# roboyu/Kimera-Multi

Measured on AMD Instinct MI355X. Metric: dpgo edges*iters/sec (+ LC candidates verified/sec in 'lcd'), higher is better.
Workload: dtype f64

## Files before the change

### kimera-multi_amd/csrc/pgo.hip

```cpp
#include <hip/hip_runtime.h>
#include <hip/hip_ext.h>
#include <rccl/rccl.h>
#include <dlfcn.h>

#include <algorithm>
#include <chrono>
#include <thread>
#include <type_traits>
#include <cmath>
#include <cstdio>
#include <cstdlib>
#include <cstring>
#include <limits>
#include <numeric>
#include <string>
#include <vector>

#include "common.h"
#include "pgo_host.h"

#ifndef KMX_HESS_PROBE
#define KMX_HESS_PROBE 0
#endif

// ... 201 lines not shown
  static constexpr int WK = RW == 10 ? 6 : 12;
  static constexpr int QS = RW == 10 ? 4 : Q;
  __device__ static __forceinline__ void load_stored(const Dev& d, size_t k, double2 a[QS]) {
    const double2* p2 = reinterpret_cast<const double2*>(d.rec + (size_t)GS * k);
#pragma unroll
    for (int i = 0; i < QS; ++i) a[i] = p2[i];
  }
  __device__ static __forceinline__ unsigned load_word(const Dev& d, size_t k) {
    static_assert(RW == 10, "compact records only");
    return (unsigned)d.rec_o[k];
  }
  __device__ static __forceinline__ int other_of(unsigned word) {
    static_assert(RW == 10, "compact records only");
    return (int)(word << 3) >> 3;
  }
  __device__ static __forceinline__ void expand(const double2 a[QS], unsigned raw, double2 q[Q]) {
    if constexpr (RW == 10) {
      const double2 a0 = a[0], a1 = a[1], a2 = a[2], a3 = a[3];
      const int other = (int)(raw << 3) >> 3;
      const unsigned big = raw >> 29;
      const double qa = a0.x, qb = a0.y, qc = a1.x;
      const double ql = sqrt(1.0 - (qa * qa + qb * qb + qc * qc));
      const double w = big == 0 ? ql : qa, x = big == 0 ? qa : (big == 1 ? ql : qb);
      const double y = big <= 1 ? qb : (big == 2 ? ql : qc), z = big == 3 ? ql : qc;
      q[0] = make_double2(w, x);
      q[1] = make_double2(y, z);
      q[2] = make_double2(a1.y, a2.x);
      q[3] = make_double2(a2.y, a3.x);
      const double wt = a3.y;
      const long long bits = (long long)(unsigned)other | (std::signbit(wt) ? (1ll << 63) : 0ll);
      q[4] = make_double2(std::fabs(wt), __longlong_as_double(bits));
    } else {
#pragma unroll
      for (int i = 0; i < Q; ++i) q[i] = a[i];
    }
// ... 473 lines not shown
__device__ __forceinline__ double inc_owner_cost(const Dev& d, const Lane& L, const double* V, const double* pub,
                                                 char* smem) {
  using SM = SmemC<R>;
  using RC = Rec<RW>;
  int* sptr = reinterpret_cast<int*>(smem + SM::ptr_off);
  double2* xs = reinterpret_cast<double2*>(smem + SM::x_off);
  const int tid = threadIdx.x;
  const int p0 = L.p0, np = L.np, K0 = L.k0, n = L.n;
  if (tid <= np) sptr[tid] = d.inc_ptr[p0 + tid] - K0;
  {
    const double2* v2 = reinterpret_cast<const double2*>(V + (size_t)p0 * 4 * R);
    for (int i = tid; i < np * 2 * R; i += BLOCK) xs[i] = v2[i];
  }
  __syncthreads();
  double cost = 0.0;
  for (int k = tid; k < n; k += BLOCK) {
    double2 q[RC::Q];
    RC::load(d, (size_t)(K0 + k), q);
    const int2 in = RC::inc(q);
    const int o = in.x;
    const bool tail = (in.y >> 31) & 1;
    if (o >= 0 && !tail) continue;
    const double2* o2 =
        reinterpret_cast<const double2*>((o >= 0) ? V + (size_t)o * 4 * R : pub + (size_t)(-1 - o) * 4 * R);
    double2 vs2[2 * R], vo2[2 * R];
#pragma unroll
    for (int i = 0; i < 2 * R; ++i) vo2[i] = o2[i];
    int lo = 0, hi = np;
    while (hi - lo > 1) {
      const int mid = (lo + hi) >> 1;
// ... 446 lines not shown

template <int R, int RW, int RM>
__device__ __forceinline__ void body_grad(const Dev& d, int gated, char* smem) {
  const Lane L = lane_map<R>(d);
  if (gated) {
    if (L.tile == 0 && threadIdx.x == 0) store_gnc(d.gnc, load_gnc(d.gnc_next));
    if (d.gnc_next->fired) {
      const int np = L.np, p0 = L.p0;
      for (int t = threadIdx.x; t < np; t += blockDim.x) pose_precond<RW>(d, p0 + t);
      __syncthreads();
    }
  }
  if (d.ctl[L.l].phase != PH_START) return;
  double y[4] = {0, 0, 0, 0}, G[4], cost = 0.0;
  hinc_grad<R, RW>(d, L, d.X, d.pub, G, &cost, smem);
  if (L.valid) load4(d.X + (size_t)L.pose * 4 * R + 4 * L.a, y);
  constexpr int NDP = R >= 5 ? 1 : 2;
  double2 dpart[NDP];
  {
    const double2* Dp2 = reinterpret_cast<const double2*>(d.hD + SYM4 * (size_t)L.pose);
#pragma unroll
    for (int u = 0; u < NDP; ++u) {
      const int i = L.a + u * R;
      dpart[u] = (L.valid && i < 5) ? Dp2[i] : make_double2(0.0, 0.0);
    }
  }
  double S[9], gr[4], zr[4];
  double* scr = reinterpret_cast<double*>(smem);
  group_symYtG<R, true>(y, G, L.base, S, scr);
#pragma unroll
  for (int c = 0; c < 3; ++c) gr[c] = G[c] - (y[0] * S[0 * 3 + c] + y[1] * S[1 * 3 + c] + y[2] * S[2 * 3 + c]);
  gr[3] = G[3];
  group_precon<R, true>(d, L.pose, L.valid, y, gr, L.base, zr, scr);
  double vals[3] = {cost, 0.0, 0.0};
  if (L.valid) {
    vals[1] = gr[0] * gr[0] + gr[1] * gr[1] + gr[2] * gr[2] + gr[3] * gr[3];
    vals[2] = zr[0] * gr[0] + zr[1] * gr[1] + zr[2] * gr[2] + zr[3] * gr[3];
  }
  finish_tile<RED_GRAD, 3, RM>(d, L, vals, smem + SmemHG<R>::red_off, [&]() {
    if (!L.valid) return;
    const size_t o = (size_t)L.pose * 4 * R + 4 * L.a;
    store4(d.g + o, gr);
    store4(d.z + o, zr);
    if (L.a == 0) {
      double* Sp = d.S + 6 * (size_t)L.pose;
      Sp[0] = S[0]; Sp[1] = S[1]; Sp[2] = S[2]; Sp[3] = S[4]; Sp[4] = S[5]; Sp[5] = S[8];
    }
    double2* Fp2 = reinterpret_cast<double2*>(d.hDS + SYM4 * (size_t)L.pose);
#pragma unroll
    for (int u = 0; u < NDP; ++u) {
      const int i = L.a + u * R;
      if (i < 5) {
        const double sx = i == 0 ? S[0] : i == 1 ? S[2] : i == 2 ? S[4] : 0.0;
        const double sy = i == 0 ? S[1] : i == 2 ? S[5] : i == 3 ? S[8] : 0.0;
        Fp2[i] = make_double2(dpart[u].x - sx, dpart[u].y - sy);
      }
    }
  });
}
// ... 700 lines not shown
      if (threadIdx.x == 0) {
        if (u.stop >= 0) d.ctl[L.l].tcg_stop = u.stop;
        d.ctl[L.l].phase = PH_STEP;
      }
    }
  }
}

template <int R>
__device__ __forceinline__ void body_commit(const Dev& d, int fold, int final) {
  const Lane L = lane_map<R>(d);
  if (final && L.tile == 0 && threadIdx.x == 0) {
    d.gnc->inner += 1;
    d.gnc->rounds += 1;
  }
  bool commit;
  if (fold) {
    __shared__ int sph;
    __shared__ Ctl cs;
    __shared__ double rl[NPART * WAVES];
    const Ctl& c = d.ctl[L.l];
    const bool writer = L.tile == L.rt0;
    if (writer && threadIdx.x < (int)(sizeof(Ctl) / 8))
      reinterpret_cast<double*>(&cs)[threadIdx.x] = reinterpret_cast<const double*>(&c)[threadIdx.x];
    if (threadIdx.x == 0) sph = c.phase;
    __syncthreads();
    if (sph != PH_STEP) return;
    RobotSum<NPART> rs;
    rs.issue(d.part, NPART, L.rt0, L.rt1);
    double tot[NPART] = {0.0, 0.0, 0.0, 0.0};
    rs.finish(d.part, NPART, rl, tot);
    if (d.p.rgd) {
      commit = true;
    } else {
      const double model_dec = -0.5 * tot[2];
      const double rho = (model_dec > 0.0) ? (c.f_cur - tot[0]) / model_dec : -1.0;
      commit = rho > d.p.accept_rho;
    }
    if (threadIdx.x == 0 && writer) {
      control_on(cs, d, L.l, RED_COST, tot, R, true);
      cs.phase = PH_STEP;
      d.ctl[L.l] = cs;
    }
  } else {
    const Ctl& c = d.ctl[L.l];
    commit = c.commit != 0;
    if (final && !commit && c.chg_acc > 0.0 && L.valid) {
      const int s = d.pose_slot[L.pose];
      if (s >= 0) {
        const size_t o = (size_t)L.pose * 4 * R + 4 * L.a;
        double v[4];
        load4(d.X + o, v);
        store4(d.pub + (size_t)s * 4 * R + 4 * L.a, v);
      }
    }
  }
  if (!commit || !L.valid) return;
  const size_t o = (size_t)L.pose * 4 * R + 4 * L.a;
  double v[4];
  load4(d.Xt + o, v);
  store4(d.X + o, v);
  if (!final) return;
  const int s = d.pose_slot[L.pose];
  if (s >= 0) store4(d.pub + (size_t)s * 4 * R + 4 * L.a, v);
}

template <int R, int RW, int RM>
__global__ __launch_bounds__(BLOCK, LB<R>::w) void k_grad(Dev d, int gated) {
  KMX_SMEM;
  body_grad<R, RW, RM>(d, gated, smem);
}
template <int R, int RW, int RM, bool GRAD, bool EARLY>
__global__ __launch_bounds__(BLOCK, LB<R>::w) void k_hess(Dev d, int gated, int slot, HostStatus* hs,
                                                          unsigned long long seq) {
// ... 515 lines not shown
  static constexpr int MAX_GROUPS = 4;
  struct Group {
    int l0 = 0, l1 = 0;
    int t0 = 0, nt = 0;
    int blind_left = 0;
  };
  int groups_req = 2;
  std::vector<Group> grp;
  Group all;
  int grm = 2;
  int grm_forced = -1;
  hipStream_t gstream[MAX_GROUPS - 1] = {nullptr, nullptr, nullptr};
  hipEvent_t ev_fork = nullptr, ev_join[MAX_GROUPS - 1] = {nullptr, nullptr, nullptr};
  bool hess_gate = true;
  bool tcg_tail = true;
  int rm = RM_LAUNCH;
  int rm_forced = -1;
  int early_stop = 1;
  int decide_forced = -1;
  bool poll_timeout = false;
  bool timing = false;
  int* d_hv_launch = nullptr;
  std::vector<hipEvent_t> ev_pool;
  size_t ev_used = 0;
  double *d_accV = nullptr, *d_accY = nullptr;
  double* d_X0 = nullptr;
  double acc_gamma = 0.0;
  int acc_k = 0;
  bool acc_ready = false, acc_started = false;
};
// ... 98 lines not shown
  p.mu_step = h->P.gnc_mu_step;
  p.rel_tol = h->gnc_rel_tol;
  p.gnc_on = h->gnc_on;
  p.inner_iters = h->gnc_inner_iters;
  p.max_updates = h->gnc_max_updates;
  p.n_ext = h->n_ext;
  p.rgd = h->P.method == KMX_METHOD_RGD ? 1 : 0;
  p.rgd_step = h->P.rgd_stepsize;
  h->dv.ext = h->d_ext;
}

void enqueue_publish(kmx_pgo* h) {
  const int ps = 4 * h->P.r;
  const long long tot = h->n_owned * ps;
  if (tot == 0) return;
  hipLaunchKernelGGL(k_publish, dim3((unsigned)((tot / 2 + 255) / 256)), dim3(256), 0, h->stream, h->d_vec,
                     h->d_pub + (size_t)h->first_owned * ps, h->d_pub_src + h->first_owned, (int)h->n_owned, ps);
}

void enqueue_precond(kmx_pgo* h, int gated) {
  const int blocks = std::max(1, std::min(gated ? 256 : 1024, (h->nloc + 127) / 128));
  with_rw(h->rw, [&](auto RW) {
    hipLaunchKernelGGL(k_precond<RW()>, dim3(blocks), dim3(128), 0, h->stream, h->dv, gated);
  });
}

bool enqueue_begin(kmx_pgo* h, const unsigned char* d_active, int mode, bool defer = false,
                   hipEvent_t done = nullptr) {
  const bool may_fire = h->P.robust_cost == KMX_COST_GNC_TLS && (h->gnc_on || (mode & BEGIN_FORCE_GNC));
  if (!may_fire) mode |= BEGIN_SOLO;
  const unsigned grid = may_fire ? 1 + (unsigned)std::min(256, std::max(1, (h->n_gnc + 255) / 256)) : 1;
// ... 189 lines not shown
    if (t.e0)
      hipExtLaunchKernelGGL((k_step<R, RW>), grid, blk, SmemF<R>::bytes, q.s, t.e0, t.e1, 0u, q.d, cin, cout, j,
                            t.slot, hs, seq);
    else
      hipLaunchKernelGGL((k_step<R, RW>), grid, blk, SmemF<R>::bytes, q.s, q.d, cin, cout, j, t.slot, hs, seq);
    if (poll && j > 0 && !wait_running(h, seq, q.l0, q.l0 + q.nl)) {
      J = j + 1;
      break;
    }
  }
  h->ctl_par = J & 1;
  tcg_polled(h, *q.st, poll, J - 1);
}

template <int R, int RW, int RM>
void enqueue_round_t(kmx_pgo* h, const unsigned char* d_active, int G) {
  constexpr bool cons = RM == RM_CONSUMER;
  const dim3 blk(BLOCK);
  const bool rgd = h->P.method == KMX_METHOD_RGD, os = cons && onesync(h);
  if (multi_rtr(h))
    (void)hipMemcpyAsync(h->d_X0, h->dv.X, sizeof(double) * (size_t)h->dv.vec, hipMemcpyDeviceToDevice, h->stream);
  const bool pend = enqueue_begin(h, d_active, BEGIN_ROUND, true, G > 1 ? h->ev_fork : nullptr);
  Chain q[kmx_pgo::MAX_GROUPS];
  if (G == 1) q[0] = make_chain(h, h->all, h->stream);
  else
    for (int g = 0; g < G; ++g) q[g] = make_chain(h, h->grp[g], g == 0 ? h->stream : h->gstream[g - 1]);
  for (int g = 1; g < G; ++g) (void)hipStreamWaitEvent(q[g].s, h->ev_fork, 0);
  const int iters = rgd ? 1 : h->P.rtr_iterations;
  const bool fgrad = fold_grad<RM>(h), fcost = fold_cost<RM>(h);
  for (int it = 0; it < iters; ++it) {
    for (int g = 0; g < G; ++g) {
// ... 12 lines not shown
      const bool last = it + 1 == iters;
      hipEvent_t join = g > 0 && last ? h->ev_join[g - 1] : nullptr;
      if (!os && !(cons && stopped[g]) && !tail_fused<RM>(h))
        hipLaunchKernelGGL((k_retract<R>), grid, blk, SmemU::bytes, q[g].s, q[g].d, cons && !rgd ? 2 : 0,
                           (const Ctl*)h->d_ctl);
      if (fcost && join)
        hipExtLaunchKernelGGL((k_cost<R, RW, RM>), grid, blk, SmemC<R>::bytes, q[g].s, nullptr, join, 0u, q[g].d, src);
      else
        hipLaunchKernelGGL((k_cost<R, RW, RM>), grid, blk, SmemC<R>::bytes, q[g].s, q[g].d, src);
      if (!fcost) red<R>(q[g], RED_COST, nullptr, 0, -1, join);
      if (!last)
        hipLaunchKernelGGL((k_commit<R>), grid, blk, 0, q[g].s, q[g].d, 0, 0);
    }
  }
  for (int g = 1; g < G; ++g) (void)hipStreamWaitEvent(h->stream, h->ev_join[g - 1], 0);
  hipLaunchKernelGGL((k_commit<R>), dim3(h->ntiles), blk, 0, h->stream, h->dv, fcost ? 1 : 0, 1);
  if (multi_rtr(h))
    hipLaunchKernelGGL(k_change, dim3(h->dv.L), blk, 0, h->stream, h->dv, (const double*)h->d_X0, 4 * R);
}

void enqueue_round(kmx_pgo* h, const unsigned char* d_active) {
  const int G = groups_in_effect(h);
  const int rm = G > 1 ? h->grm : h->rm;
  with_r(h->P.r, [&](auto R) {
    constexpr int r = decltype(R)::value;
    if (rm == RM_CONSUMER)
      with_rw(h->rw, [&](auto RW) { enqueue_round_t<r, RW(), RM_CONSUMER>(h, d_active, G); });
    else
      with_rw(h->rw, [&](auto RW) { enqueue_round_t<r, RW(), RM_LAUNCH>(h, d_active, G); });
  });
}

double accel_gamma_next(const kmx_pgo* h) {
  const double N = (double)h->n_robots;
  return (1.0 + std::sqrt(1.0 + 4.0 * N * N * h->acc_gamma * h->acc_gamma)) / (2.0 * N);
}
void launch_accel(kmx_pgo* h, double c, int mode) {
  with_r(h->P.r, [&](auto R) {
    hipLaunchKernelGGL(k_accel<R()>, dim3(h->ntiles), dim3(BLOCK), 0, h->stream, h->dv, h->d_accV, h->d_accY, c, mode);
  });
}
void enqueue_accel_pre(kmx_pgo* h) {
  if (!h->P.acceleration || h->acc_ready || h->ntiles == 0) return;
  if (!h->acc_started) {
// ... 54 lines not shown
  h->P = *params;
  h->device = device;
  hipError_t e = hipStreamCreateWithFlags(&h->stream, hipStreamNonBlocking);
  if (e != hipSuccess) {
    delete h;
    return kmx::fail(KMX_EHIP, std::string("hipStreamCreate: ") + hipGetErrorString(e));
  }
  h->own_stream = true;
  if (const char* v = std::getenv("KMX_RED")) {
    const int m = std::atoi(v);
    h->rm_forced = m == 0 ? RM_LAUNCH : m == 2 ? RM_CONSUMER : -1;
  }
  if (const char* v = std::getenv("KMX_HESS_DECIDE")) h->decide_forced = std::atoi(v) != 0 ? 1 : 0;
  if (const char* v = std::getenv("KMX_HESS_GATE")) h->hess_gate = std::atoi(v) != 0;
  if (const char* v = std::getenv("KMX_TCG_TAIL")) h->tcg_tail = std::atoi(v) != 0;
  if (const char* v = std::getenv("KMX_TCG_GROUPS")) {
    const int g = std::atoi(v);
    h->groups_req = g >= 4 ? 4 : g >= 2 ? 2 : 1;
  }
  if (const char* v = std::getenv("KMX_GROUP_RED")) h->grm_forced = std::atoi(v) == 2 ? RM_CONSUMER : RM_LAUNCH;
  for (int g = 1; g < h->groups_req && e == hipSuccess; ++g) {
    e = hipStreamCreateWithFlags(&h->gstream[g - 1], hipStreamNonBlocking);
    if (e == hipSuccess) e = hipEventCreate(&h->ev_join[g - 1]);
  }
  if (e == hipSuccess && h->groups_req > 1) e = hipEventCreate(&h->ev_fork);
  if (e != hipSuccess) {
    (void)kmx_pgo_destroy(h);
    return kmx::fail(KMX_EHIP, std::string("robot group streams: ") + hipGetErrorString(e));
  }
  *out = h;
// ... 245 lines not shown
  return KMX_OK;
  KMX_GUARD_END
}

static int check_robot(kmx_pgo* h, int robot) {
  KMX_CHECK(ready(h), KMX_ESTATE, "set_graph first");
  KMX_CHECK(robot >= 0 && robot < h->n_robots && h->local_of[robot] >= 0, KMX_EINVAL, "robot is not local");
  return 0;
}

extern "C" int kmx_pgo_set_iterate(kmx_pgo* h, int robot, const double* X) {
  if (int rc = check_robot(h, robot)) return rc;
  KMX_CHECK(X, KMX_EINVAL, "null X");
  KMX_HIP(hipSetDevice(h->device));
  const int ps = 4 * h->P.r, l = h->local_of[robot];
  KMX_HIP(hipMemcpyAsync(h->d_vec + (size_t)h->loff[l] * ps, X, sizeof(double) * h->npose[robot] * ps,
                         hipMemcpyHostToDevice, h->stream));
  KMX_HIP(hipStreamSynchronize(h->stream));
  accel_reset(h);
  return KMX_OK;
}

extern "C" int kmx_pgo_get_iterate(kmx_pgo* h, int robot, double* X) {
  if (int rc = check_robot(h, robot)) return rc;
  KMX_CHECK(X, KMX_EINVAL, "null X");
  KMX_HIP(hipSetDevice(h->device));
  const int ps = 4 * h->P.r, l = h->local_of[robot];
  KMX_HIP(hipMemcpyAsync(X, h->d_vec + (size_t)h->loff[l] * ps, sizeof(double) * h->npose[robot] * ps,
                         hipMemcpyDeviceToHost, h->stream));
  KMX_HIP(hipStreamSynchronize(h->stream));
  return KMX_OK;
}

extern "C" int kmx_pgo_public_count(kmx_pgo* h, int64_t* n_public, int64_t* first_owned, int64_t* n_owned) {
  KMX_CHECK(ready(h), KMX_ESTATE, "set_graph first");
  if (n_public) *n_public = h->npub;
  if (first_owned) *first_owned = h->first_owned;
  if (n_owned) *n_owned = h->n_owned;
  return KMX_OK;
}

extern "C" int kmx_pgo_pack_public(kmx_pgo* h, void* dev_out) {
  KMX_CHECK(ready(h), KMX_ESTATE, "set_graph first");
  KMX_CHECK(dev_out || h->n_owned == 0, KMX_EINVAL, "null device buffer");
  KMX_HIP(hipSetDevice(h->device));
  const int ps = 4 * h->P.r;
  const long long tot = h->n_owned * ps;
  if (tot)
    hipLaunchKernelGGL(k_pack, dim3((unsigned)((tot + 255) / 256)), dim3(256), 0, h->stream, h->d_vec,
                       (double*)dev_out, h->d_own_src, 0, (int)h->n_owned, ps);
  KMX_HIP(hipGetLastError());
  return KMX_OK;
}

extern "C" int kmx_pgo_unpack_public(kmx_pgo* h, const void* dev_table) {
  KMX_CHECK(ready(h), KMX_ESTATE, "set_graph first");
  KMX_CHECK(dev_table || h->npub == 0, KMX_EINVAL, "null device buffer");
  KMX_HIP(hipSetDevice(h->device));
  if (h->npub)
    KMX_HIP(hipMemcpyAsync(h->d_pub, dev_table, sizeof(double) * h->npub * 4 * h->P.r, hipMemcpyDeviceToDevice,
                           h->stream));
  return KMX_OK;
}

// ... 4 lines not shown
extern "C" int kmx_pgo_scatter_public_rows(kmx_pgo* h, const int32_t* dev_slots, int64_t n, const void* dev_rows) {
  return kmx_pgo_exchange_unpack(h, dev_slots, n, nullptr, 0, dev_rows);
}

extern "C" int kmx_pgo_exchange_pack(kmx_pgo* h, const int32_t* dev_slots, int64_t n, const int32_t* dev_seg,
                                     int n_seg, void* dev_out) {
  KMX_CHECK(ready(h), KMX_ESTATE, "set_graph first");
  KMX_CHECK(n >= 0 && n_seg >= 0 && n_seg <= 1024 && (n == 0 || (dev_slots && dev_out)) &&
                (n_seg == 0 || (dev_seg && dev_out)),
            KMX_EINVAL, "bad argument");
  KMX_HIP(hipSetDevice(h->device));
  enqueue_accel_pre(h);
  const int ps = 4 * h->P.r;
  const long long tot = (long long)n * ps + n_seg;
  if (tot)
    hipLaunchKernelGGL(k_gather_slots, dim3((unsigned)((tot + 255) / 256)), dim3(256), 0, h->stream, h->d_vec,
                       h->d_pub_src, (const int*)dev_slots, (long long)n, (int)h->npub, (double*)dev_out, ps,
                       (const int*)dev_seg, n_seg, (const double*)h->d_relc, h->dv.L);
  KMX_HIP(hipGetLastError());
  return KMX_OK;
}

extern "C" int kmx_pgo_exchange_unpack(kmx_pgo* h, const int32_t* dev_slots, int64_t n, const int32_t* dev_seg,
                                       int n_seg, const void* dev_in) {
  KMX_CHECK(ready(h), KMX_ESTATE, "set_graph first");
  KMX_CHECK(n >= 0 && n_seg >= 0 && n_seg <= 1024 && (n == 0 || (dev_slots && dev_in)) &&
                (n_seg == 0 || (dev_seg && dev_in)),
            KMX_EINVAL, "bad argument");
  KMX_HIP(hipSetDevice(h->device));
  const int ps = 4 * h->P.r;
  if (n_seg > h->ext_cap) {
// ... 25 lines not shown
  const auto t0 = std::chrono::steady_clock::now();
  while (r == ncclInProgress) {
    if (std::chrono::steady_clock::now() - t0 > std::chrono::seconds(60))
      return kmx::fail(KMX_EHIP, std::string(what) + ": still in progress after 60 s");
    std::this_thread::yield();
    if (ncclCommGetAsyncError(h->comm, &r) != ncclSuccess) r = ncclSystemError;
  }
  if (r != ncclSuccess) return kmx::fail(KMX_EHIP, std::string(what) + ": " + ncclGetErrorString(r));
  return KMX_OK;
}

int enqueue_exchange(kmx_pgo* h) {
  if (!h->xchg) return KMX_OK;
  const int ps = 4 * h->P.r, W = h->world;
  const long long ts = h->xn_send * ps + W, tr = h->xn_recv * ps + W;
  hipLaunchKernelGGL(k_xgather, dim3((unsigned)((ts + 255) / 256)), dim3(256), 0, h->stream, h->d_vec,
                     h->d_pub_src, h->d_xs_slots, h->d_xs_rseg, h->xn_send, h->d_xsbuf, ps, h->d_xs_seg, W,
                     (const double*)h->d_relc, h->dv.L);
  KMX_NCCL(ncclGroupStart());
  for (int q = 0; q < W; ++q) {
    if (q == h->rank && !h->xchg_self_p2p) continue;
    KMX_NCCL(ncclSend(h->d_xsbuf + h->xs_off[q], (size_t)h->xs_cnt[q], ncclDouble, q, h->comm, h->stream));
    KMX_NCCL(ncclRecv(h->d_xrbuf + h->xr_off[q], (size_t)h->xr_cnt[q], ncclDouble, q, h->comm, h->stream));
  }
  if (int rc = nccl_settle(h, ncclGroupEnd(), "ncclGroupEnd")) return rc;
  if (!h->xchg_self_p2p)
    KMX_HIP(hipMemcpyAsync(h->d_xrbuf + h->xr_off[h->rank], h->d_xsbuf + h->xs_off[h->rank],
                           sizeof(double) * h->xs_cnt[h->rank], hipMemcpyDeviceToDevice, h->stream));
  hipLaunchKernelGGL(k_xscatter, dim3((unsigned)((tr + 255) / 256)), dim3(256), 0, h->stream, h->d_pub,
                     h->d_xr_slots, h->d_xr_rseg, h->xn_recv, (const double*)h->d_xrbuf, ps, h->d_xr_seg, W, h->d_ext);
  if (h->n_ext != W) {
// ... 223 lines not shown

extern "C" int kmx_pgo_iterate(kmx_pgo* h, const uint8_t* active, kmx_iter_stats* stats) {
  KMX_GUARD_BEGIN
  KMX_CHECK(ready(h), KMX_ESTATE, "set_graph first");
  KMX_CHECK(active, KMX_EINVAL, "null active mask");
  KMX_HIP(hipSetDevice(h->device));
  const int L = (int)h->robots.size();
  std::vector<unsigned char> act(L);
  for (int l = 0; l < L; ++l) act[l] = active[h->robots[l]] ? 1 : 0;
  if (h->P.acceleration)
    for (int l = 0; l < L; ++l)
      KMX_CHECK(act[l], KMX_EUNSUP, "acceleration needs every local robot active (concurrent schedule)");
  KMX_HIP(hipMemcpyAsync(h->d_active, act.data(), L, hipMemcpyHostToDevice, h->stream));
  enqueue_accel_pre(h);
  if (int rc = enqueue_exchange(h)) return rc;
  enqueue_round(h, h->d_active);
  enqueue_accel_post(h);
  KMX_HIP(hipGetLastError());
  std::vector<Ctl> ctl(L);
  KMX_HIP(hipMemcpyAsync(ctl.data(), h->d_ctl, sizeof(Ctl) * L, hipMemcpyDeviceToHost, h->stream));
  KMX_HIP(hipStreamSynchronize(h->stream));
  std::vector<unsigned char> ones(L, 1);
  KMX_HIP(hipMemcpyAsync(h->d_active, ones.data(), L, hipMemcpyHostToDevice, h->stream));
  KMX_HIP(hipStreamSynchronize(h->stream));
  if (stats) {
    for (int a = 0; a < h->n_robots; ++a) std::memset(&stats[a], 0, sizeof(kmx_iter_stats));
    for (int l = 0; l < L; ++l) {
      const Ctl& c = ctl[l];
      kmx_iter_stats& s = stats[h->robots[l]];
      s.updated = c.updated;
      s.tcg_iterations = c.tcg_iter;
// ... 9 lines not shown
      s.hessvecs = c.hessvecs;
    }
  }
  return KMX_OK;
  KMX_GUARD_END
}

extern "C" int kmx_pgo_iterate_async(kmx_pgo* h, int rounds, int refresh_local) {
  KMX_CHECK(ready(h), KMX_ESTATE, "set_graph first");
  KMX_CHECK(rounds >= 0, KMX_EINVAL, "negative rounds");
  KMX_HIP(hipSetDevice(h->device));
  if (refresh_local && rounds > 0) enqueue_publish(h);
  for (int i = 0; i < rounds; ++i) {
    enqueue_accel_pre(h);
    if (int rc = enqueue_exchange(h)) return rc;
    enqueue_round(h, h->d_active);
    enqueue_accel_post(h);
  }
  KMX_HIP(hipGetLastError());
  return KMX_OK;
}

extern "C" int kmx_pgo_sync(kmx_pgo* h) {
  KMX_CHECK(h, KMX_EINVAL, "null handle");
  KMX_HIP(hipSetDevice(h->device));
  KMX_HIP(hipStreamSynchronize(h->stream));
  return KMX_OK;
}

extern "C" int kmx_pgo_set_gnc_schedule(kmx_pgo* h, int enabled, int inner_iters, int max_updates,
                                        double rel_change_tol) {
// ... 147 lines not shown
  return KMX_OK;
}

extern "C" int kmx_pgo_get_trajectory(kmx_pgo* h, int robot, const double* anchor, double* out) {
  KMX_GUARD_BEGIN
  if (int rc = check_robot(h, robot)) return rc;
  KMX_CHECK(anchor && out, KMX_EINVAL, "null argument");
  KMX_HIP(hipSetDevice(h->device));
  const int ps = 4 * h->P.r, l = h->local_of[robot], n = h->npose[robot];
  if (int rc = ensure_scratch(h, (size_t)ps + (size_t)std::max(n, 1) * 12)) return rc;
  double* d_anchor = h->d_scratch;
  double* d_out = h->d_scratch + ps;
  KMX_HIP(hipMemcpyAsync(d_anchor, anchor, sizeof(double) * ps, hipMemcpyHostToDevice, h->stream));
  if (n)
    hipLaunchKernelGGL(k_traj, dim3((n + 127) / 128), dim3(128), 0, h->stream,
                       (const double*)(h->d_vec + (size_t)h->loff[l] * ps), n, h->P.r, (const double*)d_anchor, d_out);
  KMX_HIP(hipGetLastError());
  KMX_HIP(hipMemcpyAsync(out, d_out, sizeof(double) * n * 12, hipMemcpyDeviceToHost, h->stream));
  KMX_HIP(hipStreamSynchronize(h->stream));
  return KMX_OK;
  KMX_GUARD_END
}

extern "C" int kmx_pgo_eval(kmx_pgo* h, int robot, int mode, const double* V, double* out, double* scalar) {
  KMX_GUARD_BEGIN
  if (int rc = check_robot(h, robot)) return rc;
  KMX_CHECK(mode >= KMX_EVAL_COST_EGRAD && mode <= KMX_EVAL_RETRACT, KMX_EINVAL, "bad eval mode");
  KMX_CHECK(out && (V || mode == KMX_EVAL_RGRAD), KMX_EINVAL, "null argument");
  KMX_HIP(hipSetDevice(h->device));
  const int ps = 4 * h->P.r, l = h->local_of[robot], n = h->npose[robot];
  const size_t vec = (size_t)std::max(h->nloc, 1) * ps;
// ... 104 lines not shown
```

### kimera-multi_amd/csrc/pgo_check.cpp

```cpp
#include <climits>
#include <cstdio>
#include <string>
#include <vector>

#include "pgo_host.h"

namespace {

int g_fail = 0;

#define CHECK(cond)                                                     \
  do {                                                                  \
    if (!(cond)) {                                                      \
      std::fprintf(stderr, "pgo_check.cpp:%d: %s\n", __LINE__, #cond);  \
      ++g_fail;                                                         \
    }                                                                   \
  } while (0)

struct Rot {
  double m[9];
};
Rot rot(int axis, double a, bool half_turn = false) {
  const double c = half_turn ? -1.0 : std::cos(a), s = half_turn ? 0.0 : std::sin(a);
  switch (axis) {
// ... 155 lines not shown
  const RecAt want[11] = {{0, 0, 1, 1},  {1, 5, 1, 2},  {2, 0, 0, 0},  {3, 1, 1, 2}, {4, 4, 0, -4}, {5, 1, 0, 1},
                          {6, 3, 1, -3}, {7, 5, 0, 0},  {8, 2, 1, 4},  {9, 3, 0, -2}, {10, 2, 0, 3}};
  const int GS = kmx::rec_gs(p.rw);
  CHECK(GS == (full ? 16 : 8));
  CHECK(p.rec.size() == (size_t)12 * GS);
  CHECK(p.rec_o.size() == (full ? (size_t)1 : (size_t)12));
  if (p.rec.size() != (size_t)12 * GS || p.rec_o.size() != (full ? (size_t)1 : (size_t)12)) return;
  for (const RecAt& w : want) {
    const double* c = &p.rec[(size_t)w.pos * GS];
    const int64_t e = p.loc_edge_gid[w.k];
    const double wk = g.weight[e] * g.kappa[e], wt = g.weight[e] * g.tau[e];
    if (!full) {
      const unsigned word = (unsigned)p.rec_o[w.pos];
      CHECK(((int)(word << 3) >> 3) == w.other);
      double q[4], Rq[9];
      kmx::quat_unpack(c, (int)(word >> 29), q);
      kmx::quat_to_rot(q, Rq);
      for (int i = 0; i < 9; ++i) CHECK(std::fabs(Rq[i] - g.R[9 * e + i]) <= 1e-12);
      for (int i = 0; i < 3; ++i) CHECK(c[3 + i] == g.t[3 * e + i]);
      CHECK(c[6] == wk && std::fabs(c[7]) == wt);
      CHECK(std::signbit(c[7]) == (w.tail != 0));
    } else {
      for (int i = 0; i < 9; ++i) CHECK(c[i] == g.R[9 * e + i]);
      for (int i = 0; i < 3; ++i) CHECK(c[9 + i] == g.t[3 * e + i]);
      CHECK(c[12] == wk && c[13] == wt);
      uint64_t bits;
      std::memcpy(&bits, &c[14], 8);
      CHECK((int)(uint32_t)bits == w.other);
      CHECK((int)((bits >> 32) & 0x7fffffffu) == w.k);
      CHECK((bits >> 63) == (uint64_t)w.tail);
      CHECK(c[15] == 0.0);
// ... 225 lines not shown
```

### kimera-multi_amd/csrc/pgo_host.h

```cpp
#pragma once
#include <algorithm>
#include <climits>
#include <cmath>
#include <cstdint>
#include <cstdlib>
#include <cstring>
#include <string>
#include <vector>

#include "kmx_abi.h"

namespace kmx {

constexpr int WAVES = 4;
constexpr int tile_poses(int r, int w = WAVES) { return w * (64 / r); }
constexpr int TILES_TARGET = 736;

enum RedMode { RM_LAUNCH = 0, RM_CONSUMER = 2 };
constexpr int RM_CONSUMER_MAX_POSES = 80000;
constexpr int GROUP_CONSUMER_MAX_TILES = 384;

constexpr int rec_gs(int rw) { return rw == 10 ? 8 : 16; }

struct alignas(16) TileDesc {
// ... 208 lines not shown
  const int GS = rec_gs(RW);
  g.rec.assign((size_t)((int64_t)g.ninc + 1) * GS, 0.0);
  g.rec_o.assign(RW == 10 ? (size_t)g.ninc + 1 : 1, 0);
  g.eipos.assign(std::max(g.mloc, 1), PgoInt2{-1, -1});
  std::vector<int> fill(inc_ptr.begin(), inc_ptr.end() - 1);
  auto put_rec = [&](int pos, int k, int64_t e, int other, int code) {
    double* c = &g.rec[(size_t)pos * GS];
    const double* Q = RW == 10 ? &quat[3 * (size_t)k] : R + 9 * e;
    int j = 0;
    for (int q = 0; q < (RW == 10 ? 3 : 9); ++q) c[j++] = Q[q];
    for (int q = 0; q < 3; ++q) c[j++] = t[3 * e + q];
    c[j++] = weight[e] * kappa[e];
    const double wt = weight[e] * tau[e];
    if (RW == 10) {
      c[j++] = (code & 0x80000000) ? -wt : wt;
      g.rec_o[pos] = (int)(((unsigned)other & 0x1fffffffu) | ((unsigned)qbig[k] << 29));
    } else {
      c[j++] = wt;
      const long long bits = (long long)(unsigned)other | (long long)((unsigned long long)(unsigned)code << 32);
      std::memcpy(&c[j], &bits, 8);
    }
  };
  for (int k = 0; k < g.mloc; ++k) {
    const int64_t e = ledges[k];
    const bool priv = r1[e] == r2[e];
    if (g.local_of[r1[e]] >= 0) {
      const int sp = lpose(r1[e], p1[e]);
      const int other = priv ? lpose(r2[e], p2[e]) : (int)(-1 - slot_of(r2[e], p2[e]));
      g.eipos[k].x = fill[sp];
      put_rec(fill[sp]++, k, e, other, (int)(k | 0x80000000u));
    }
// ... 130 lines not shown
```

Measured before the change: 1.058 billion.

## Pack tail bit into record word, swap X/Xt on commit, reuse smem pose data

After: 1.057 billion. No clear change (-0.1%).

```diff
diff --git a/kimera-multi_amd/csrc/pgo.hip b/kimera-multi_amd/csrc/pgo.hip
--- a/kimera-multi_amd/csrc/pgo.hip
+++ b/kimera-multi_amd/csrc/pgo.hip
@@ -239,11 +239,15 @@
     static_assert(RW == 10, "compact records only");
     return (int)(word << 3) >> 3;
   }
+  __device__ static __forceinline__ bool tail_of(unsigned word) {
+    static_assert(RW == 10, "compact records only");
+    return (word >> 31) != 0;
+  }
   __device__ static __forceinline__ void expand(const double2 a[QS], unsigned raw, double2 q[Q]) {
     if constexpr (RW == 10) {
       const double2 a0 = a[0], a1 = a[1], a2 = a[2], a3 = a[3];
       const int other = (int)(raw << 3) >> 3;
-      const unsigned big = raw >> 29;
+      const unsigned big = (raw >> 29) & 3u;
       const double qa = a0.x, qb = a0.y, qc = a1.x;
       const double ql = sqrt(1.0 - (qa * qa + qb * qb + qc * qc));
       const double w = big == 0 ? ql : qa, x = big == 0 ? qa : (big == 1 ? ql : qb);
@@ -747,6 +751,53 @@
   }
   __syncthreads();
   double cost = 0.0;
+  if constexpr (RW == 10) {
+    constexpr int NI = 2;
+    for (int kb = tid; kb < n; kb += NI * BLOCK) {
+      unsigned w[NI];
+#pragma unroll
+      for (int i = 0; i < NI; ++i) {
+        const int k = kb + i * BLOCK;
+        w[i] = k < n ? RC::load_word(d, (size_t)(K0 + k)) : 0u;
+      }
+#pragma unroll
+      for (int i = 0; i < NI; ++i) {
+        const int k = kb + i * BLOCK;
+        const int o = RC::other_of(w[i]);
+        const bool tail = RC::tail_of(w[i]);
+        if (o >= 0 && !tail) continue;
+        double2 qs[RC::QS], vs2[2 * R], vo2[2 * R];
+        RC::load_stored(d, (size_t)(K0 + k), qs);
+        const double2* o2 =
+            reinterpret_cast<const double2*>((o >= 0) ? V + (size_t)o * 4 * R : pub + (size_t)(-1 - o) * 4 * R);
+#pragma unroll
+        for (int u = 0; u < 2 * R; ++u) vo2[u] = o2[u];
+        int lo = 0, hi = np;
+        while (hi - lo > 1) {
+          const int mid = (lo + hi) >> 1;
+          if (sptr[mid] <= k) lo = mid;
+          else hi = mid;
+        }
+        const double2* s2 = xs + lo * 2 * R;
+#pragma unroll
+        for (int u = 0; u < 2 * R; ++u) vs2[u] = s2[u];
+        double2 q[RC::Q];
+        RC::expand(qs, w[i], q);
+        Edge E;
+        RC::edge(q, E);
+        double c = 0.0;
+#pragma unroll
+        for (int a = 0; a < R; ++a) {
+          const double vs[4] = {vs2[2 * a].x, vs2[2 * a].y, vs2[2 * a + 1].x, vs2[2 * a + 1].y};
+          const double vo[4] = {vo2[2 * a].x, vo2[2 * a].y, vo2[2 * a + 1].x, vo2[2 * a + 1].y};
+          double dummy[4] = {0.0, 0.0, 0.0, 0.0};
+          c += incidence_row(E, tail, vs, vo, dummy);
+        }
+        cost += c;
+      }
+    }
+    return cost;
+  }
   for (int k = tid; k < n; k += BLOCK) {
     double2 q[RC::Q];
     RC::load(d, (size_t)(K0 + k), q);
@@ -1223,7 +1274,15 @@
   if (d.ctl[L.l].phase != PH_START) return;
   double y[4] = {0, 0, 0, 0}, G[4], cost = 0.0;
   hinc_grad<R, RW>(d, L, d.X, d.pub, G, &cost, smem);
-  if (L.valid) load4(d.X + (size_t)L.pose * 4 * R + 4 * L.a, y);
+  static_assert(SCR_BYTES <= SmemHG<R>::x_off, "scratch");
+  if constexpr (RW != 10) {
+    if (L.valid) load4(d.X + (size_t)L.pose * 4 * R + 4 * L.a, y);
+  } else if (L.valid) {
+    const double2* s2 =
+        reinterpret_cast<const double2*>(smem + SmemHG<R>::x_off) + ((L.pose - L.p0) * R + L.a) * 2;
+    const double2 sa = s2[0], sb = s2[1];
+    y[0] = sa.x; y[1] = sa.y; y[2] = sb.x; y[3] = sb.y;
+  }
   constexpr int NDP = R >= 5 ? 1 : 2;
   double2 dpart[NDP];
   {
@@ -1251,7 +1310,7 @@
     const size_t o = (size_t)L.pose * 4 * R + 4 * L.a;
     store4(d.g + o, gr);
     store4(d.z + o, zr);
-    if (L.a == 0) {
+    if (L.a == 0 && d.hz) {
       double* Sp = d.S + 6 * (size_t)L.pose;
       Sp[0] = S[0]; Sp[1] = S[1]; Sp[2] = S[2]; Sp[3] = S[4]; Sp[4] = S[5]; Sp[5] = S[8];
     }
@@ -1982,7 +2041,8 @@
     d.gnc->inner += 1;
     d.gnc->rounds += 1;
   }
-  bool commit;
+  const bool swap = final == 2;
+  bool commit = false, moved = false;
   if (fold) {
     __shared__ int sph;
     __shared__ Ctl cs;
@@ -1993,39 +2053,53 @@
       reinterpret_cast<double*>(&cs)[threadIdx.x] = reinterpret_cast<const double*>(&c)[threadIdx.x];
     if (threadIdx.x == 0) sph = c.phase;
     __syncthreads();
-    if (sph != PH_STEP) return;
-    RobotSum<NPART> rs;
-    rs.issue(d.part, NPART, L.rt0, L.rt1);
-    double tot[NPART] = {0.0, 0.0, 0.0, 0.0};
-    rs.finish(d.part, NPART, rl, tot);
-    if (d.p.rgd) {
-      commit = true;
-    } else {
-      const double model_dec = -0.5 * tot[2];
-      const double rho = (model_dec > 0.0) ? (c.f_cur - tot[0]) / model_dec : -1.0;
-      commit = rho > d.p.accept_rho;
-    }
-    if (threadIdx.x == 0 && writer) {
-      control_on(cs, d, L.l, RED_COST, tot, R, true);
-      cs.phase = PH_STEP;
-      d.ctl[L.l] = cs;
+    if (sph == PH_STEP) {
+      RobotSum<NPART> rs;
+      rs.issue(d.part, NPART, L.rt0, L.rt1);
+      double tot[NPART] = {0.0, 0.0, 0.0, 0.0};
+      rs.finish(d.part, NPART, rl, tot);
+      if (d.p.rgd) {
+        commit = true;
+      } else {
+        const double model_dec = -0.5 * tot[2];
+        const double rho = (model_dec > 0.0) ? (c.f_cur - tot[0]) / model_dec : -1.0;
+        commit = rho > d.p.accept_rho;
+      }
+      if (threadIdx.x == 0 && writer) {
+        control_on(cs, d, L.l, RED_COST, tot, R, true);
+        cs.phase = PH_STEP;
+        d.ctl[L.l] = cs;
+      }
     }
   } else {
     const Ctl& c = d.ctl[L.l];
     commit = c.commit != 0;
-    if (final && !commit && c.chg_acc > 0.0 && L.valid) {
-      const int s = d.pose_slot[L.pose];
-      if (s >= 0) {
-        const size_t o = (size_t)L.pose * 4 * R + 4 * L.a;
-        double v[4];
-        load4(d.X + o, v);
-        store4(d.pub + (size_t)s * 4 * R + 4 * L.a, v);
-      }
-    }
-  }
-  if (!commit || !L.valid) return;
+    moved = final && !commit && c.chg_acc > 0.0;
+  }
+  if (!L.valid) return;
   const size_t o = (size_t)L.pose * 4 * R + 4 * L.a;
   double v[4];
+  if (swap) {
+    const int s = d.pose_slot[L.pose];
+    if (commit) {
+      if (s < 0) return;
+      load4(d.Xt + o, v);
+    } else {
+      load4(d.X + o, v);
+      store4(d.Xt + o, v);
+      if (!moved || s < 0) return;
+    }
+    store4(d.pub + (size_t)s * 4 * R + 4 * L.a, v);
+    return;
+  }
+  if (moved) {
+    const int s = d.pose_slot[L.pose];
+    if (s >= 0) {
+      load4(d.X + o, v);
+      store4(d.pub + (size_t)s * 4 * R + 4 * L.a, v);
+    }
+  }
+  if (!commit) return;
   load4(d.Xt + o, v);
   store4(d.X + o, v);
   if (!final) return;
@@ -2571,6 +2645,7 @@
   hipEvent_t ev_fork = nullptr, ev_join[MAX_GROUPS - 1] = {nullptr, nullptr, nullptr};
   bool hess_gate = true;
   bool tcg_tail = true;
+  bool commit_swap = true;
   int rm = RM_LAUNCH;
   int rm_forced = -1;
   int early_stop = 1;
@@ -2699,7 +2774,7 @@
   const int ps = 4 * h->P.r;
   const long long tot = h->n_owned * ps;
   if (tot == 0) return;
-  hipLaunchKernelGGL(k_publish, dim3((unsigned)((tot / 2 + 255) / 256)), dim3(256), 0, h->stream, h->d_vec,
+  hipLaunchKernelGGL(k_publish, dim3((unsigned)((tot / 2 + 255) / 256)), dim3(256), 0, h->stream, h->dv.X,
                      h->d_pub + (size_t)h->first_owned * ps, h->d_pub_src + h->first_owned, (int)h->n_owned, ps);
 }
 
@@ -2919,7 +2994,7 @@
 }
 
 template <int R, int RW, int RM>
-void enqueue_round_t(kmx_pgo* h, const unsigned char* d_active, int G) {
+void enqueue_round_t(kmx_pgo* h, const unsigned char* d_active, int G, bool swap) {
   constexpr bool cons = RM == RM_CONSUMER;
   const dim3 blk(BLOCK);
   const bool rgd = h->P.method == KMX_METHOD_RGD, os = cons && onesync(h);
@@ -2962,20 +3037,22 @@
     }
   }
   for (int g = 1; g < G; ++g) (void)hipStreamWaitEvent(h->stream, h->ev_join[g - 1], 0);
-  hipLaunchKernelGGL((k_commit<R>), dim3(h->ntiles), blk, 0, h->stream, h->dv, fcost ? 1 : 0, 1);
+  hipLaunchKernelGGL((k_commit<R>), dim3(h->ntiles), blk, 0, h->stream, h->dv, fcost ? 1 : 0, swap ? 2 : 1);
+  if (swap) std::swap(h->dv.X, h->dv.Xt);
   if (multi_rtr(h))
     hipLaunchKernelGGL(k_change, dim3(h->dv.L), blk, 0, h->stream, h->dv, (const double*)h->d_X0, 4 * R);
 }
 
-void enqueue_round(kmx_pgo* h, const unsigned char* d_active) {
+void enqueue_round(kmx_pgo* h, const unsigned char* d_active, bool all_active) {
   const int G = groups_in_effect(h);
   const int rm = G > 1 ? h->grm : h->rm;
+  const bool swap = all_active && h->commit_swap;
   with_r(h->P.r, [&](auto R) {
     constexpr int r = decltype(R)::value;
     if (rm == RM_CONSUMER)
-      with_rw(h->rw, [&](auto RW) { enqueue_round_t<r, RW(), RM_CONSUMER>(h, d_active, G); });
+      with_rw(h->rw, [&](auto RW) { enqueue_round_t<r, RW(), RM_CONSUMER>(h, d_active, G, swap); });
     else
-      with_rw(h->rw, [&](auto RW) { enqueue_round_t<r, RW(), RM_LAUNCH>(h, d_active, G); });
+      with_rw(h->rw, [&](auto RW) { enqueue_round_t<r, RW(), RM_LAUNCH>(h, d_active, G, swap); });
   });
 }
 
@@ -3060,6 +3137,7 @@
   if (const char* v = std::getenv("KMX_HESS_DECIDE")) h->decide_forced = std::atoi(v) != 0 ? 1 : 0;
   if (const char* v = std::getenv("KMX_HESS_GATE")) h->hess_gate = std::atoi(v) != 0;
   if (const char* v = std::getenv("KMX_TCG_TAIL")) h->tcg_tail = std::atoi(v) != 0;
+  if (const char* v = std::getenv("KMX_COMMIT_SWAP")) h->commit_swap = std::atoi(v) != 0;
   if (const char* v = std::getenv("KMX_TCG_GROUPS")) {
     const int g = std::atoi(v);
     h->groups_req = g >= 4 ? 4 : g >= 2 ? 2 : 1;
@@ -3335,7 +3413,7 @@
   KMX_CHECK(X, KMX_EINVAL, "null X");
   KMX_HIP(hipSetDevice(h->device));
   const int ps = 4 * h->P.r, l = h->local_of[robot];
-  KMX_HIP(hipMemcpyAsync(h->d_vec + (size_t)h->loff[l] * ps, X, sizeof(double) * h->npose[robot] * ps,
+  KMX_HIP(hipMemcpyAsync(h->dv.X + (size_t)h->loff[l] * ps, X, sizeof(double) * h->npose[robot] * ps,
                          hipMemcpyHostToDevice, h->stream));
   KMX_HIP(hipStreamSynchronize(h->stream));
   accel_reset(h);
@@ -3347,7 +3425,7 @@
   KMX_CHECK(X, KMX_EINVAL, "null X");
   KMX_HIP(hipSetDevice(h->device));
   const int ps = 4 * h->P.r, l = h->local_of[robot];
-  KMX_HIP(hipMemcpyAsync(X, h->d_vec + (size_t)h->loff[l] * ps, sizeof(double) * h->npose[robot] * ps,
+  KMX_HIP(hipMemcpyAsync(X, h->dv.X + (size_t)h->loff[l] * ps, sizeof(double) * h->npose[robot] * ps,
                          hipMemcpyDeviceToHost, h->stream));
   KMX_HIP(hipStreamSynchronize(h->stream));
   return KMX_OK;
@@ -3368,7 +3446,7 @@
   const int ps = 4 * h->P.r;
   const long long tot = h->n_owned * ps;
   if (tot)
-    hipLaunchKernelGGL(k_pack, dim3((unsigned)((tot + 255) / 256)), dim3(256), 0, h->stream, h->d_vec,
+    hipLaunchKernelGGL(k_pack, dim3((unsigned)((tot + 255) / 256)), dim3(256), 0, h->stream, h->dv.X,
                        (double*)dev_out, h->d_own_src, 0, (int)h->n_owned, ps);
   KMX_HIP(hipGetLastError());
   return KMX_OK;
@@ -3403,7 +3481,7 @@
   const int ps = 4 * h->P.r;
   const long long tot = (long long)n * ps + n_seg;
   if (tot)
-    hipLaunchKernelGGL(k_gather_slots, dim3((unsigned)((tot + 255) / 256)), dim3(256), 0, h->stream, h->d_vec,
+    hipLaunchKernelGGL(k_gather_slots, dim3((unsigned)((tot + 255) / 256)), dim3(256), 0, h->stream, h->dv.X,
                        h->d_pub_src, (const int*)dev_slots, (long long)n, (int)h->npub, (double*)dev_out, ps,
                        (const int*)dev_seg, n_seg, (const double*)h->d_relc, h->dv.L);
   KMX_HIP(hipGetLastError());
@@ -3459,7 +3537,7 @@
   if (!h->xchg) return KMX_OK;
   const int ps = 4 * h->P.r, W = h->world;
   const long long ts = h->xn_send * ps + W, tr = h->xn_recv * ps + W;
-  hipLaunchKernelGGL(k_xgather, dim3((unsigned)((ts + 255) / 256)), dim3(256), 0, h->stream, h->d_vec,
+  hipLaunchKernelGGL(k_xgather, dim3((unsigned)((ts + 255) / 256)), dim3(256), 0, h->stream, h->dv.X,
                      h->d_pub_src, h->d_xs_slots, h->d_xs_rseg, h->xn_send, h->d_xsbuf, ps, h->d_xs_seg, W,
                      (const double*)h->d_relc, h->dv.L);
   KMX_NCCL(ncclGroupStart());
@@ -3713,7 +3791,7 @@
   KMX_HIP(hipMemcpyAsync(h->d_active, act.data(), L, hipMemcpyHostToDevice, h->stream));
   enqueue_accel_pre(h);
   if (int rc = enqueue_exchange(h)) return rc;
-  enqueue_round(h, h->d_active);
+  enqueue_round(h, h->d_active, std::all_of(act.begin(), act.end(), [](unsigned char a) { return a != 0; }));
   enqueue_accel_post(h);
   KMX_HIP(hipGetLastError());
   std::vector<Ctl> ctl(L);
@@ -3753,7 +3831,7 @@
   for (int i = 0; i < rounds; ++i) {
     enqueue_accel_pre(h);
     if (int rc = enqueue_exchange(h)) return rc;
-    enqueue_round(h, h->d_active);
+    enqueue_round(h, h->d_active, true);
     enqueue_accel_post(h);
   }
   KMX_HIP(hipGetLastError());
@@ -3931,7 +4009,7 @@
   KMX_HIP(hipMemcpyAsync(d_anchor, anchor, sizeof(double) * ps, hipMemcpyHostToDevice, h->stream));
   if (n)
     hipLaunchKernelGGL(k_traj, dim3((n + 127) / 128), dim3(128), 0, h->stream,
-                       (const double*)(h->d_vec + (size_t)h->loff[l] * ps), n, h->P.r, (const double*)d_anchor, d_out);
+                       (const double*)(h->dv.X + (size_t)h->loff[l] * ps), n, h->P.r, (const double*)d_anchor, d_out);
   KMX_HIP(hipGetLastError());
   KMX_HIP(hipMemcpyAsync(out, d_out, sizeof(double) * n * 12, hipMemcpyDeviceToHost, h->stream));
   KMX_HIP(hipStreamSynchronize(h->stream));
diff --git a/kimera-multi_amd/csrc/pgo_check.cpp b/kimera-multi_amd/csrc/pgo_check.cpp
--- a/kimera-multi_amd/csrc/pgo_check.cpp
+++ b/kimera-multi_amd/csrc/pgo_check.cpp
@@ -193,7 +193,7 @@
       const unsigned word = (unsigned)p.rec_o[w.pos];
       CHECK(((int)(word << 3) >> 3) == w.other);
       double q[4], Rq[9];
-      kmx::quat_unpack(c, (int)(word >> 29), q);
+      kmx::quat_unpack(c, (int)((word >> 29) & 3u), q);
       kmx::quat_to_rot(q, Rq);
       for (int i = 0; i < 9; ++i) CHECK(std::fabs(Rq[i] - g.R[9 * e + i]) <= 1e-12);
       for (int i = 0; i < 3; ++i) CHECK(c[3 + i] == g.t[3 * e + i]);
diff --git a/kimera-multi_amd/csrc/pgo_host.h b/kimera-multi_amd/csrc/pgo_host.h
--- a/kimera-multi_amd/csrc/pgo_host.h
+++ b/kimera-multi_amd/csrc/pgo_host.h
@@ -246,7 +246,7 @@
     const double wt = weight[e] * tau[e];
     if (RW == 10) {
       c[j++] = (code & 0x80000000) ? -wt : wt;
-      g.rec_o[pos] = (int)(((unsigned)other & 0x1fffffffu) | ((unsigned)qbig[k] << 29));
+      g.rec_o[pos] = (int)(((unsigned)other & 0x1fffffffu) | ((unsigned)qbig[k] << 29) | ((unsigned)code & 0x80000000u));
     } else {
       c[j++] = wt;
       const long long bits = (long long)(unsigned)other | (long long)((unsigned long long)(unsigned)code << 32);
diff --git a/kimera-multi_amd/csrc/pgo_word_check.cpp b/kimera-multi_amd/csrc/pgo_word_check.cpp
--- /dev/null
+++ b/kimera-multi_amd/csrc/pgo_word_check.cpp
@@ -0,0 +1,177 @@
+#include <cmath>
+#include <cstdio>
+#include <string>
+#include <vector>
+
+#include "pgo_host.h"
+
+namespace {
+
+int g_fail = 0;
+
+#define CHECK(cond)                                                          \
+  do {                                                                       \
+    if (!(cond)) {                                                           \
+      std::fprintf(stderr, "pgo_word_check.cpp:%d: %s\n", __LINE__, #cond);  \
+      ++g_fail;                                                              \
+    }                                                                        \
+  } while (0)
+
+struct Lcg {
+  uint64_t s;
+  uint32_t next() {
+    s = s * 6364136223846793005ull + 1442695040888963407ull;
+    return (uint32_t)(s >> 33);
+  }
+  int below(int n) { return (int)(next() % (uint32_t)n); }
+  double unit() { return (next() + 0.5) / 2147483648.0; }
+};
+
+int other_of(unsigned word) { return (int)(word << 3) >> 3; }
+
+struct Team {
+  std::vector<int32_t> n_poses;
+  std::vector<uint8_t> local;
+  std::vector<int32_t> r1, p1, r2, p2;
+  std::vector<double> R, t, kappa, tau, weight;
+  std::vector<uint8_t> fixed;
+};
+
+void quat_rot(const double* q4, double* R) {
+  const double n = std::sqrt(q4[0] * q4[0] + q4[1] * q4[1] + q4[2] * q4[2] + q4[3] * q4[3]);
+  const double q[4] = {q4[0] / n, q4[1] / n, q4[2] / n, q4[3] / n};
+  kmx::quat_to_rot(q, R);
+}
+
+Team random_team(uint64_t seed, bool full) {
+  Lcg rng{seed};
+  Team g;
+  const int nr = 4;
+  g.n_poses = {9, 17, 0, 23};
+  g.local = {0, 1, 1, 1};
+  auto edge = [&](int a, int i, int b, int j, int big_want) {
+    g.r1.push_back(a); g.p1.push_back(i); g.r2.push_back(b); g.p2.push_back(j);
+    double q[4];
+    for (int c = 0; c < 4; ++c) q[c] = (rng.unit() - 0.5) * 0.9;
+    q[big_want] = (rng.below(2) ? 1.0 : -1.0) * (1.0 + rng.unit());
+    double Rm[9];
+    quat_rot(q, Rm);
+    g.R.insert(g.R.end(), Rm, Rm + 9);
+    for (int c = 0; c < 3; ++c) g.t.push_back(rng.unit() * 4.0 - 2.0);
+    g.kappa.push_back(1.0 + rng.unit());
+    g.tau.push_back(1.0 + rng.unit());
+    g.weight.push_back(rng.below(5) == 0 ? 0.0 : rng.unit());
+    g.fixed.push_back((uint8_t)rng.below(2));
+  };
+  for (int a = 0; a < nr; ++a)
+    for (int p = 0; p + 1 < g.n_poses[a]; ++p) edge(a, p, a, p + 1, rng.below(4));
+  for (int e = 0; e < 120; ++e) {
+    int a = rng.below(nr), b = rng.below(nr);
+    if (g.n_poses[a] == 0 || g.n_poses[b] == 0) continue;
+    const int i = rng.below(g.n_poses[a]), j = rng.below(g.n_poses[b]);
+    if (a == b && i == j) continue;
+    edge(a, i, b, j, e % 4);
+  }
+  if (full) g.R[9 * 10 + 1] += 1e-6;
+  return g;
+}
+
+void check_team(uint64_t seed, bool full) {
+  const Team g = random_team(seed, full);
+  kmx::PgoPlanIn in;
+  in.r = 5;
+  kmx::PgoPlan p;
+  std::string err;
+  const int64_t m = (int64_t)g.r1.size();
+  const int rc = kmx::pgo_plan(in, (int)g.n_poses.size(), g.n_poses.data(), g.local.data(), m, g.r1.data(),
+                               g.p1.data(), g.r2.data(), g.p2.data(), g.R.data(), g.t.data(), g.kappa.data(),
+                               g.tau.data(), g.weight.data(), g.fixed.data(), &p, &err);
+  CHECK(rc == KMX_OK);
+  if (rc != KMX_OK) {
+    std::fprintf(stderr, "seed %llu: %s\n", (unsigned long long)seed, err.c_str());
+    return;
+  }
+  CHECK(p.rw == (full ? 16 : 10));
+  if (full) {
+    CHECK(p.rec_o.size() == 1 && p.rec_o[0] == 0);
+    return;
+  }
+  CHECK(p.rec_o.size() == (size_t)p.ninc + 1);
+  CHECK(p.rec.size() == ((size_t)p.ninc + 1) * 8);
+  if (p.rec_o.size() != (size_t)p.ninc + 1 || p.rec.size() != ((size_t)p.ninc + 1) * 8) return;
+  std::vector<int> loff(g.n_poses.size(), -1);
+  int nloc = 0;
+  for (size_t a = 0; a < g.n_poses.size(); ++a)
+    if (g.local[a]) { loff[a] = nloc; nloc += g.n_poses[a]; }
+  std::vector<int64_t> keys;
+  for (int64_t e = 0; e < m; ++e)
+    if (g.r1[e] != g.r2[e]) {
+      keys.push_back(((int64_t)g.r1[e] << 32) | (uint32_t)g.p1[e]);
+      keys.push_back(((int64_t)g.r2[e] << 32) | (uint32_t)g.p2[e]);
+    }
+  std::sort(keys.begin(), keys.end());
+  keys.erase(std::unique(keys.begin(), keys.end()), keys.end());
+  auto endpoint = [&](int64_t e, int rb, int pp) {
+    if (g.r1[e] == g.r2[e]) return loff[rb] + pp;
+    const int64_t k = ((int64_t)rb << 32) | (uint32_t)pp;
+    return (int)(-1 - (std::lower_bound(keys.begin(), keys.end(), k) - keys.begin()));
+  };
+  std::vector<char> seen((size_t)p.ninc + 1, 0);
+  int tails = 0, heads = 0, bigs[4] = {0, 0, 0, 0}, zero_tails = 0;
+  int k = 0;
+  for (int64_t e = 0; e < m; ++e) {
+    const bool l1 = g.local[g.r1[e]] != 0, l2 = g.local[g.r2[e]] != 0;
+    if (!l1 && !l2) continue;
+    CHECK(k < p.mloc && p.loc_edge_gid[k] == e);
+    double q4[4], q3[3];
+    kmx::rot_to_quat(&g.R[9 * e], q4);
+    const int big = kmx::quat_pack(q4, q3);
+    const double wt = g.weight[e] * g.tau[e];
+    for (int side = 0; side < 2; ++side) {
+      const bool tail = side == 0;
+      if (!(tail ? l1 : l2)) {
+        CHECK((tail ? p.eipos[k].x : p.eipos[k].y) == -1);
+        continue;
+      }
+      const int pos = tail ? p.eipos[k].x : p.eipos[k].y;
+      CHECK(pos >= 0 && pos < p.ninc);
+      if (pos < 0 || pos >= p.ninc) continue;
+      CHECK(!seen[pos]);
+      seen[pos] = 1;
+      const unsigned word = (unsigned)p.rec_o[pos];
+      const double stored = p.rec[(size_t)pos * 8 + 7];
+      const int other = tail ? endpoint(e, g.r2[e], g.p2[e]) : endpoint(e, g.r1[e], g.p1[e]);
+      CHECK((word >> 31) == (tail ? 1u : 0u));
+      CHECK(((word >> 31) != 0) == std::signbit(stored));
+      CHECK(std::fabs(stored) == wt);
+      CHECK((word & 0x7fffffffu) == (((unsigned)other & 0x1fffffffu) | ((unsigned)big << 29)));
+      CHECK(other_of(word) == other);
+      CHECK((int)((word >> 29) & 3u) == big);
+      const bool owner_word = other_of(word) < 0 || (word >> 31) != 0;
+      const bool owner_edge = g.r1[e] != g.r2[e] || tail;
+      CHECK(owner_word == owner_edge);
+      tail ? ++tails : ++heads;
+      ++bigs[big];
+      if (tail && wt == 0.0) ++zero_tails;
+    }
+    ++k;
+  }
+  CHECK(k == p.mloc);
+  for (int pos = 0; pos < p.ninc; ++pos) CHECK(seen[pos]);
+  CHECK(p.rec_o[p.ninc] == 0);
+  CHECK(tails > 0 && heads > 0 && zero_tails > 0);
+  for (int b = 0; b < 4; ++b) CHECK(bigs[b] > 0);
+}
+
+}
+
+int main() {
+  for (uint64_t seed = 1; seed <= 8; ++seed) check_team(seed, false);
+  check_team(3, true);
+  if (g_fail) {
+    std::fprintf(stderr, "pgo_word_check: %d failure(s)\n", g_fail);
+    return 1;
+  }
+  std::printf("pgo_word_check ok\n");
+  return 0;
+}
```
